# EmaMule/2D-to-3D-Style-Transfer

Measured on AMD Instinct MI355X. Metric: style-transfer iters/sec (512x512, 8 views, cow_mesh), higher is better.
Workload: dtype f32; 1 GPU; BASELINE.json configs[1]: cow_mesh + Style_1, 512x512, 8 views/GPU/iter, texture-only optimisation, white backgrounds (second_approach loop body); texture=512x512, targets_hoisted=content renders + content features + style Grams, parallelism=views sharded dp1, RCCL all-reduce of the texture gradient

## Files before the change

2d-to-3d-style-transfer_amd/csrc/flat.hip:

```cpp
#include "common.h"

namespace {

typedef unsigned u32x4 __attribute__((ext_vector_type(4)));
typedef unsigned u32x2 __attribute__((ext_vector_type(2)));

__global__ __launch_bounds__(256) void flat_v0_kernel(const float *__restrict__ img, const float *__restrict__ color, int S,
                                                      int total4, uint8_t *__restrict__ v0) {
    const int i = blockIdx.x * 256 + threadIdx.x;
    if (i >= total4) return;
    const int per = (S * S) >> 2;
    const int n = i / per, r = i - n * per;
    u32x4 d = u32x4{0u, 0u, 0u, 0u};
#pragma unroll
    for (int c = 0; c < 3; ++c) {
        const u32x4 q = *reinterpret_cast<const u32x4 *>(img + ((size_t)(n * 3 + c) * per + r) * 4);
        d |= q ^ __float_as_uint(color[c]);
    }
    reinterpret_cast<unsigned *>(v0)[i] = (d[0] ? 1u : 0u) | (d[1] ? 0x100u : 0u) | (d[2] ? 0x10000u : 0u) | (d[3] ? 0x1000000u : 0u);
}

__global__ __launch_bounds__(256) void flat_v2_kernel(const uint8_t *__restrict__ v0, int S, int total4, uint8_t *__restrict__ v2) {
    const int i = blockIdx.x * 256 + threadIdx.x;
    if (i >= total4) return;
    const int Sh = S >> 1, q4 = Sh >> 2;
    const int x4 = i % q4, y = (i / q4) % Sh, n = i / (q4 * Sh);
    const int c0 = 8 * x4;
    unsigned w[4] = {0u, 0u, 0u, 0u};
#pragma unroll
    for (int dy = -2; dy <= 5; ++dy) {
        const int yy = 4 * (y >> 1) + dy;
        if (yy < 0 || yy >= S) continue;
        const uint8_t *row = v0 + ((size_t)n * S + yy) * S + c0;
        const u32x2 m = *reinterpret_cast<const u32x2 *>(row);
        w[1] |= m[0]; w[2] |= m[1];
        if (c0 > 0) w[0] |= *reinterpret_cast<const unsigned *>(row - 4);
        if (c0 + 8 < S) w[3] |= *reinterpret_cast<const unsigned *>(row + 8);
    }
    unsigned out = 0;
#pragma unroll
    for (int pr = 0; pr < 2; ++pr) {
        unsigned any = 0;
#pragma unroll
        for (int k = 4 * pr + 2; k <= 4 * pr + 9; ++k) any |= (w[k >> 2] >> (8 * (k & 3))) & 0xffu;
        out |= (any ? 0x0101u : 0u) << (16 * pr);
    }
    reinterpret_cast<unsigned *>(v2)[i] = out;
}

struct FlatGeo {
    int tiles_x, tiles_y, rows, cols;
};

__global__ __launch_bounds__(256) void flat_flags_kernel(const uint8_t *__restrict__ v2, int S, FlatGeo g1, FlatGeo g2, int t1, int t2,
                                                         int total, uint8_t *__restrict__ flags) {
    const int i = blockIdx.x * 4 + (threadIdx.x >> 6), lane = threadIdx.x & 63;
    if (i >= total) return;
    const int Sh = S >> 1;
    const int launch = i < t1 ? 0 : (i < t1 + t2 ? 1 : 2);
    const FlatGeo g = launch == 0 ? FlatGeo{g1.tiles_x, g1.tiles_y, g1.rows >> 1, g1.cols >> 1} : g2;
    const int t = launch == 0 ? i : (launch == 1 ? i - t1 : i - t1 - t2);
    const int per_img = g.tiles_x * g.tiles_y;
    const int n = t / per_img, r = t - n * per_img;
    const int ty = r / g.tiles_x, tx = r - ty * g.tiles_x;
    const int x0 = tx * g.cols, y0 = ty * g.rows;
    const int margin = launch == 0 ? 0 : (launch == 1 ? 1 : 5);
    const int ya = max(0, y0 - margin), yb = min(Sh - 1, y0 + g.rows - 1 + margin);
    const int xa = max(0, x0 - margin), xb = min(Sh - 1, x0 + g.cols - 1 + margin);
    const int w = xb - xa + 1, count = (yb - ya + 1) * w;
    const uint8_t *base = v2 + (size_t)n * Sh * Sh;
    unsigned any = 0;
    for (int k = lane; k < count; k += 64) {
        const int y = ya + k / w, x = xa + k % w;
        any |= base[(size_t)y * Sh + x];
    }
    const bool vary = __any(any != 0);
    if (lane == 0) flags[i] = vary ? 1 : 0;
}

struct FlatLists {
    int *list[3], *map[3];
};

__global__ __launch_bounds__(1024) void flat_lists_kernel(const uint8_t *__restrict__ flags, FlatGeo g1, FlatGeo g2, int t1, int t2,
                                                          FlatLists out, int *__restrict__ counts) {
    __shared__ int scan[1024];
    __shared__ int rep[81];
    const int launch = blockIdx.x, tid = threadIdx.x;
    const uint8_t *__restrict__ f = flags + (launch == 0 ? 0 : (launch == 1 ? t1 : t1 + t2));
    const FlatGeo g = launch == 0 ? g1 : g2;
    const int total = launch == 0 ? t1 : t2;
    int *__restrict__ list = out.list[launch];
    int *__restrict__ map = out.map[launch];
    const int per = (total + 1023) / 1024;
    const int lo = min(total, tid * per), hi = min(total, lo + per);
    struct Walk { int ty, tx; };
    const int r0 = lo % (g.tiles_x * g.tiles_y);
    const Walk w0{r0 / g.tiles_x, r0 % g.tiles_x};
    auto cls = [&](const Walk &w) {
        return ((min(w.ty, 2) * 3 + min(g.tiles_y - 1 - w.ty, 2)) * 3 + min(w.tx, 2)) * 3 + min(g.tiles_x - 1 - w.tx, 2);
    };
    auto step = [&](Walk &w) {
        if (++w.tx == g.tiles_x) { w.tx = 0; if (++w.ty == g.tiles_y) w.ty = 0; }
    };
    unsigned long long fm = 0;
    if (per <= 64)
        for (int t = lo; t < hi; ++t) fm |= (unsigned long long)(f[t] ? 1 : 0) << (t - lo);
    auto varying = [&](int t) { return per <= 64 ? (int)((fm >> (t - lo)) & 1ull) : (int)f[t]; };
    if (tid < 81) rep[tid] = 0x7fffffff;
    __syncthreads();
    Walk w = w0;
    for (int t = lo; t < hi; ++t, step(w)) {
        const int c = cls(w);
        if (!varying(t) && t < *(volatile int *)&rep[c]) atomicMin(&rep[c], t);
    }
    __syncthreads();
    int cnt = 0;
    w = w0;
    for (int t = lo; t < hi; ++t, step(w)) cnt += (varying(t) || rep[cls(w)] == t) ? 1 : 0;
    scan[tid] = cnt;
    __syncthreads();
    for (int d = 1; d < 1024; d <<= 1) {
        const int v = tid >= d ? scan[tid - d] : 0;
        __syncthreads();
        scan[tid] += v;
        __syncthreads();
    }
    int o = scan[tid] - cnt;
    w = w0;
    for (int t = lo; t < hi; ++t, step(w)) {
        const int rp = rep[cls(w)];
        const bool listed = varying(t) || rp == t;
        if (listed) list[o++] = t;
        map[t] = listed ? -1 : rp;
    }
    if (tid == 1023) counts[launch] = scan[1023];
}

struct FillTile { int n, y, x; };
__device__ __forceinline__ void fill_block(char *__restrict__ base, int esize, int C, int c0, int Hh, int Ww, int br, int bc,
                                           FillTile dst, FillTile src, int tid) {
    const int row_chunks = (bc * esize) >> 4;
    const int chunks = 16 * br * row_chunks;
    for (int k = tid; k < chunks; k += 256) {
        const int q = k % row_chunks, r = (k / row_chunks) % br, c = c0 + k / (row_chunks * br);
        const size_t so = ((((size_t)src.n * C + c) * Hh + src.y * br + r) * Ww + src.x * bc) * esize + 16 * q;
        const size_t d_o = ((((size_t)dst.n * C + c) * Hh + dst.y * br + r) * Ww + dst.x * bc) * esize + 16 * q;
        *reinterpret_cast<u32x4 *>(base + d_o) = *reinterpret_cast<const u32x4 *>(base + so);
    }
}

__global__ __launch_bounds__(256) void flat_fill_kernel(const int *__restrict__ map, float *__restrict__ y, float *__restrict__ yp,
                                                        uint8_t *__restrict__ yidx, int C, int H, int W, FlatGeo g, int total) {
    const int t = blockIdx.x;
    const int rp = map[t];
    if (rp < 0 || rp >= total) return;
    const int per_img = g.tiles_x * g.tiles_y;
    const int tr = t % per_img, rr = rp % per_img;
    const FillTile dst{t / per_img, tr / g.tiles_x, tr % g.tiles_x}, src{rp / per_img, rr / g.tiles_x, rr % g.tiles_x};
    const int c0 = blockIdx.y * 16, tid = threadIdx.x;
    if (y) fill_block(reinterpret_cast<char *>(y), 4, C, c0, H, W, g.rows, g.cols, dst, src, tid);
    if (yp) fill_block(reinterpret_cast<char *>(yp), 4, C, c0, H >> 1, W >> 1, g.rows >> 1, g.cols >> 1, dst, src, tid);
    if (yidx) fill_block(reinterpret_cast<char *>(yidx), 1, C, c0, H >> 1, W >> 1, g.rows >> 1, g.cols >> 1, dst, src, tid);
}

int geo_of(int H, int W, FlatGeo *g) {
    int rows = 0, cols = 0;
    if (!st3d_wino43_tile_geometry(H, W, &rows, &cols)) return 0;
    *g = FlatGeo{W / cols, H / rows, rows, cols};
    return 1;
}

}

extern "C" int st3d_flat_levels(int S) { return (S >= 64 && (S % 64) == 0) ? 3 : 0; }

extern "C" int st3d_flat_tiles(int N, int S, int launch) {
    FlatGeo g;
    if (N <= 0 || st3d_flat_levels(S) == 0 || launch < 0 || launch > 2) return 0;
    const int R = launch == 0 ? S : S / 2;
    if (!geo_of(R, R, &g)) return 0;
    return N * g.tiles_x * g.tiles_y;
}

extern "C" size_t st3d_flat_workspace_bytes(int N, int S) {
    if (N <= 0 || st3d_flat_levels(S) == 0) return 0;
    return (size_t)N * S * S + (size_t)N * (S / 2) * (S / 2) + (size_t)st3d_flat_tiles(N, S, 0) + 2 * (size_t)st3d_flat_tiles(N, S, 1);
}

extern "C" int st3d_flat_build(const float *imgs, const float *color, int N, int S, int levels, void *workspace, size_t workspace_bytes,
                               int *list1, int *map1, int *list2, int *map2, int *list3, int *map3, int *counts, st3d_stream_t stream) {
    ST3D_CHECK_ARG(imgs && color && workspace && counts && N > 0);
    ST3D_CHECK_ARG(levels >= 1 && levels <= st3d_flat_levels(S));
    ST3D_CHECK_ARG(((uintptr_t)imgs & 15) == 0 && ((uintptr_t)workspace & 15) == 0);
    ST3D_CHECK_ARG((long)N * S * S < (1L << 31));
    ST3D_CHECK_ARG(workspace_bytes >= st3d_flat_workspace_bytes(N, S));
    ST3D_CHECK_ARG(list1 && map1 && (levels < 2 || (list2 && map2)) && (levels < 3 || (list3 && map3)));
    hipStream_t s = st3d::as_stream(stream);
    FlatGeo g1, g2;
    geo_of(S, S, &g1);
    geo_of(S / 2, S / 2, &g2);
    const int t1 = N * g1.tiles_x * g1.tiles_y, t2 = N * g2.tiles_x * g2.tiles_y;
    uint8_t *v0 = reinterpret_cast<uint8_t *>(workspace);
    uint8_t *v2 = v0 + (size_t)N * S * S;
    uint8_t *flags = v2 + (size_t)N * (S / 2) * (S / 2);
    const int n0 = N * S * S / 4, n2 = N * (S / 2) * (S / 2) / 4;
    flat_v0_kernel<<<st3d::cdiv(n0, 256), 256, 0, s>>>(imgs, color, S, n0, v0);
    ST3D_LAUNCH_CHECK();
    flat_v2_kernel<<<st3d::cdiv(n2, 256), 256, 0, s>>>(v0, S, n2, v2);
    ST3D_LAUNCH_CHECK();
    const int total = t1 + (levels - 1) * t2;
    flat_flags_kernel<<<st3d::cdiv(total, 4), 256, 0, s>>>(v2, S, g1, g2, t1, t2, total, flags);
    ST3D_LAUNCH_CHECK();
    FlatLists out{{list1, list2, list3}, {map1, map2, map3}};
    flat_lists_kernel<<<levels, 1024, 0, s>>>(flags, g1, g2, t1, t2, out, counts);
    ST3D_LAUNCH_CHECK();
    return ST3D_OK;
}

extern "C" int st3d_flat_fill(const int *tile_map, float *y, float *y_pooled, uint8_t *pool_idx, int N, int C, int H, int W,
                              st3d_stream_t stream) {
    ST3D_CHECK_ARG(tile_map && (y || y_pooled) && (!pool_idx || y_pooled));
    ST3D_CHECK_ARG(N > 0 && C > 0 && (C % 16) == 0);
    ST3D_CHECK_ARG((((uintptr_t)y | (uintptr_t)y_pooled | (uintptr_t)pool_idx) & 15) == 0);
    FlatGeo g;
    ST3D_CHECK_ARG(geo_of(H, W, &g));
    const long total = (long)N * g.tiles_x * g.tiles_y;
    ST3D_CHECK_ARG(total < (1L << 31) && C / 16 < 65536);
    flat_fill_kernel<<<dim3((unsigned)total, (unsigned)(C / 16)), 256, 0, st3d::as_stream(stream)>>>(tile_map, y, y_pooled, pool_idx, C, H,
                                                                                                  W, g, (int)total);
    ST3D_LAUNCH_CHECK();
    return ST3D_OK;
}
```

2d-to-3d-style-transfer_amd/csrc/loss.hip:

```cpp
#include "common.h"

namespace {

constexpr int NPART = 1024;

__device__ __forceinline__ float wave_sum(float v) {
#pragma unroll
    for (int o = 32; o > 0; o >>= 1) v += __shfl_down(v, o, 64);
    return v;
}

__device__ __forceinline__ void block_store_partial(float v, float *partials) {
    __shared__ float s[4];
    v = wave_sum(v);
    if ((threadIdx.x & 63) == 0) s[threadIdx.x >> 6] = v;
    __syncthreads();
    if (threadIdx.x == 0) partials[blockIdx.x] = (s[0] + s[1]) + (s[2] + s[3]);
}

__global__ __launch_bounds__(256) void sqdiff_kernel(const float *__restrict__ a, const float *__restrict__ b, size_t n,
                                                     size_t nb, float *__restrict__ D, float *__restrict__ partials) {
    float acc = 0.f;
    const size_t stride = (size_t)gridDim.x * blockDim.x;
    for (size_t i = (size_t)blockIdx.x * blockDim.x + threadIdx.x; i < n; i += stride) {
        const float d = a[i] - b[nb == n ? i : i % nb];
        if (D) D[i] = d;
        acc += d * d;
    }
    block_store_partial(acc, partials);
}

__global__ __launch_bounds__(256) void finish_kernel(const float *__restrict__ partials, int np, float scale,
                                                     float *__restrict__ out) {
    __shared__ double s[256];
    double v = 0.0;
    for (int i = threadIdx.x; i < np; i += 256) v += (double)partials[i];
    s[threadIdx.x] = v;
    __syncthreads();
    for (int o = 128; o > 0; o >>= 1) {
        if ((int)threadIdx.x < o) s[threadIdx.x] += s[threadIdx.x + o];
        __syncthreads();
    }
    if (threadIdx.x == 0) out[0] = out[0] + (float)(s[0] * (double)scale);
}

struct MultiArgs {
    const float *a[8]; const float *b[8]; float *D[8];
    size_t n[8], nb[8];
    float scale[8];
    int slot[8], first_block[9], count;
};

__global__ __launch_bounds__(256) void sqdiff_multi_kernel(const MultiArgs m, float *__restrict__ partials) {
    int k = 0;
    while (k + 1 < m.count && (int)blockIdx.x >= m.first_block[k + 1]) ++k;
    const int lb = blockIdx.x - m.first_block[k], gsz = m.first_block[k + 1] - m.first_block[k];
    const float *a = m.a[k], *b = m.b[k];
    float *D = m.D[k];
    const size_t n = m.n[k], nb = m.nb[k];
    float acc = 0.f;
    const size_t stride = (size_t)gsz * blockDim.x;
    for (size_t i = (size_t)lb * blockDim.x + threadIdx.x; i < n; i += stride) {
        const float d = a[i] - b[nb == n ? i : i % nb];
        if (D) D[i] = d;
        acc += d * d;
    }
    __shared__ float s[4];
    acc = wave_sum(acc);
    if ((threadIdx.x & 63) == 0) s[threadIdx.x >> 6] = acc;
    __syncthreads();
    if (threadIdx.x == 0) partials[(size_t)k * NPART + lb] = (s[0] + s[1]) + (s[2] + s[3]);
}

__global__ __launch_bounds__(256) void finish_multi_kernel(const MultiArgs m, const float *__restrict__ partials, float *__restrict__ out,
                                                           int zero_first, int combine, float sw, float cw) {
    __shared__ double s[256];
    __shared__ float acc3[3];
    if (threadIdx.x < 3) acc3[threadIdx.x] = zero_first ? 0.f : out[threadIdx.x];
    __syncthreads();
    for (int k = 0; k < m.count; ++k) {
        const int np = m.first_block[k + 1] - m.first_block[k];
        double v = 0.0;
        for (int i = threadIdx.x; i < np; i += 256) v += (double)partials[(size_t)k * NPART + i];
        s[threadIdx.x] = v;
        __syncthreads();
        for (int o = 128; o > 0; o >>= 1) {
            if ((int)threadIdx.x < o) s[threadIdx.x] += s[threadIdx.x + o];
            __syncthreads();
        }
        if (threadIdx.x == 0) acc3[m.slot[k]] = acc3[m.slot[k]] + (float)(s[0] * (double)m.scale[k]);
        __syncthreads();
    }
    if (threadIdx.x == 0) {
        if (combine) acc3[0] = cw * acc3[1] + sw * acc3[2];
        out[0] = acc3[0]; out[1] = acc3[1]; out[2] = acc3[2];
    }
}

__global__ __launch_bounds__(256) void axpy_diff_kernel(const float *__restrict__ a, const float *__restrict__ b, size_t n,
                                                        float coef, int accumulate, int gate, float *__restrict__ g) {
    const size_t stride = (size_t)gridDim.x * blockDim.x;
    for (size_t i = (size_t)blockIdx.x * blockDim.x + threadIdx.x; i < n; i += stride) {
        const float ai = a[i];
        const float v = coef * (ai - b[i]);
        const float t = accumulate ? g[i] + v : v;
        g[i] = (gate && ai <= 0.f) ? 0.f : t;
    }
}

__global__ __launch_bounds__(256) void masked_mse_kernel(const float *__restrict__ r, const float *__restrict__ t,
                                                         const float *__restrict__ m, int B, size_t HW, float coef,
                                                         float *__restrict__ gr, float *__restrict__ partials) {
    float acc = 0.f;
    const size_t n = (size_t)B * 3 * HW;
    const size_t stride = (size_t)gridDim.x * blockDim.x;
    for (size_t i = (size_t)blockIdx.x * blockDim.x + threadIdx.x; i < n; i += stride) {
        const size_t b = i / (3 * HW), p = i % HW;
        const float mk = m[b * HW + p];
        const float d = r[i] * mk - t[i] * mk;
        acc += d * d;
        if (gr) gr[i] = coef * d * mk;
    }
    block_store_partial(acc, partials);
}

__global__ __launch_bounds__(256) void adam_kernel(float *__restrict__ p, const float *__restrict__ g,
                                                   float *__restrict__ m, float *__restrict__ v, size_t n,
                                                   float step_size, float bc2_sqrt, float b1, float b2, float eps) {
    const size_t stride = (size_t)gridDim.x * blockDim.x;
    for (size_t i = (size_t)blockIdx.x * blockDim.x + threadIdx.x; i < n; i += stride) {
        const float gi = g[i];
        const float mi = m[i] + (gi - m[i]) * (1.0f - b1);
        const float vi = v[i] * b2 + (1.0f - b2) * gi * gi;
        m[i] = mi;
        v[i] = vi;
        const float denom = sqrtf(vi) / bc2_sqrt + eps;
        p[i] = p[i] - step_size * (mi / denom);
    }
}


__global__ __launch_bounds__(256) void tv_kernel(const float *__restrict__ img, const float *__restrict__ mask, int B, int C,
                                                 int H, int W, float *__restrict__ partials) {
    float acc = 0.f, macc = 0.f;
    const size_t HW = (size_t)H * W, n = (size_t)B * C * HW;
    const size_t stride = (size_t)gridDim.x * blockDim.x;
    for (size_t i = (size_t)blockIdx.x * blockDim.x + threadIdx.x; i < n; i += stride) {
        const size_t bc = i / HW, p = i - bc * HW, b = bc / C;
        const int y = (int)(p / W), x = (int)(p - (size_t)y * W);
        const float *mb = mask + b * HW;
        const float a = img[i], m = mb[p];
        if (y + 1 < H) acc += fabsf(a - img[i + W]) * (m * mb[p + W]);
        if (x + 1 < W) acc += fabsf(a - img[i + 1]) * (m * mb[p + 1]);
        if (bc - b * C == 0) macc += m;
    }
    __shared__ float s2[4];
    macc = wave_sum(macc);
    if ((threadIdx.x & 63) == 0) s2[threadIdx.x >> 6] = macc;
    block_store_partial(acc, partials);
    if (threadIdx.x == 0) partials[NPART + blockIdx.x] = (s2[0] + s2[1]) + (s2[2] + s2[3]);
}

__global__ __launch_bounds__(256) void tv_finish_kernel(const float *__restrict__ partials, int np, float *__restrict__ out) {
    __shared__ double s[256], sm[256];
    double v = 0.0, m = 0.0;
    for (int i = threadIdx.x; i < np; i += 256) { v += (double)partials[i]; m += (double)partials[NPART + i]; }
    s[threadIdx.x] = v; sm[threadIdx.x] = m;
    __syncthreads();
    for (int o = 128; o > 0; o >>= 1) {
        if ((int)threadIdx.x < o) { s[threadIdx.x] += s[threadIdx.x + o]; sm[threadIdx.x] += sm[threadIdx.x + o]; }
        __syncthreads();
    }
    if (threadIdx.x == 0) { out[0] = (float)(s[0] / sm[0]); out[1] = (float)sm[0]; }
}

__device__ __forceinline__ float sgn(float v) { return v > 0.f ? 1.f : (v < 0.f ? -1.f : 0.f); }

__global__ __launch_bounds__(256) void tv_grad_kernel(const float *__restrict__ img, const float *__restrict__ mask, int B, int C,
                                                      int H, int W, const float *__restrict__ loss_and_msum,
                                                      float *__restrict__ g) {
    const size_t HW = (size_t)H * W, n = (size_t)B * C * HW;
    const float inv = 1.0f / loss_and_msum[1];
    const size_t stride = (size_t)gridDim.x * blockDim.x;
    for (size_t i = (size_t)blockIdx.x * blockDim.x + threadIdx.x; i < n; i += stride) {
        const size_t bc = i / HW, p = i - bc * HW, b = bc / C;
        const int y = (int)(p / W), x = (int)(p - (size_t)y * W);
        const float *mb = mask + b * HW;
        const float a = img[i], m = mb[p];
        float d = 0.f;
        if (y + 1 < H) d += sgn(a - img[i + W]) * (m * mb[p + W]);
        if (y > 0) d -= sgn(img[i - W] - a) * (mb[p - W] * m);
        if (x + 1 < W) d += sgn(a - img[i + 1]) * (m * mb[p + 1]);
        if (x > 0) d -= sgn(img[i - 1] - a) * (mb[p - 1] * m);
        g[i] = d * inv;
    }
}

__global__ __launch_bounds__(256) void range_kernel(const float *__restrict__ t, size_t n, float *__restrict__ g,
                                                    float *__restrict__ partials) {
    float acc = 0.f;
    const size_t stride = (size_t)gridDim.x * blockDim.x;
    for (size_t i = (size_t)blockIdx.x * blockDim.x + threadIdx.x; i < n; i += stride) {
        const float v = t[i];
        acc += __builtin_elementwise_maximum(v - 1.0f, 0.f) + __builtin_elementwise_maximum(-v, 0.f);
        if (g) g[i] = v > 1.0f ? 1.0f : (v < 0.f ? -1.0f : 0.f);
    }
    block_store_partial(acc, partials);
}

inline int grid_for(size_t n) {
    size_t b = (n + 255) / 256;
    return (int)(b < 1 ? 1 : (b > NPART ? NPART : b));
}

}

extern "C" int st3d_reduce_partials(void) { return NPART; }

int st3d::finish_partials(const float *partials, int np, float scale, float *loss_out, hipStream_t stream) {
    finish_kernel<<<1, 256, 0, stream>>>(partials, np, scale, loss_out);
    ST3D_LAUNCH_CHECK();
    return ST3D_OK;
}

extern "C" int st3d_sqdiff_sum(const float *a, const float *b, size_t n, size_t nb, float scale, float *D, float *partials,
                               float *loss_out, st3d_stream_t stream) {
    ST3D_CHECK_ARG(a && b && partials && loss_out);
    ST3D_CHECK_ARG(n > 0 && nb > 0 && n % nb == 0);
    hipStream_t s = st3d::as_stream(stream);
    const int gsz = grid_for(n);
    sqdiff_kernel<<<gsz, 256, 0, s>>>(a, b, n, nb, D, partials);
    ST3D_LAUNCH_CHECK();
    finish_kernel<<<1, 256, 0, s>>>(partials, gsz, scale, loss_out);
    ST3D_LAUNCH_CHECK();
    return ST3D_OK;
}

extern "C" int st3d_sqdiff_sum_multi(const st3d_sqdiff_item *items, int count, float *partials, float *loss_out3, int zero_first,
                                     int combine, float style_weight, float content_weight, st3d_stream_t stream) {
    ST3D_CHECK_ARG(items && partials && loss_out3 && count > 0 && count <= 8);
    MultiArgs m;
    memset(&m, 0, sizeof(m));
    m.count = count;
    for (int k = 0; k < count; ++k) {
        ST3D_CHECK_ARG(items[k].a && items[k].b && items[k].n > 0 && items[k].nb > 0 && items[k].n % items[k].nb == 0);
        ST3D_CHECK_ARG(items[k].slot >= 0 && items[k].slot <= 2);
        m.a[k] = items[k].a; m.b[k] = items[k].b; m.D[k] = items[k].D;
        m.n[k] = items[k].n; m.nb[k] = items[k].nb; m.scale[k] = items[k].scale; m.slot[k] = items[k].slot;
        m.first_block[k + 1] = m.first_block[k] + grid_for(items[k].n);
    }
    hipStream_t s = st3d::as_stream(stream);
    sqdiff_multi_kernel<<<m.first_block[count], 256, 0, s>>>(m, partials);
    ST3D_LAUNCH_CHECK();
    finish_multi_kernel<<<1, 256, 0, s>>>(m, partials, loss_out3, zero_first, combine, style_weight, content_weight);
    ST3D_LAUNCH_CHECK();
    return ST3D_OK;
}

extern "C" int st3d_axpy_diff(const float *a, const float *b, size_t n, float coef, int accumulate, float *g,
                              st3d_stream_t stream) {
    ST3D_CHECK_ARG(a && b && g && n > 0);
    axpy_diff_kernel<<<grid_for(n), 256, 0, st3d::as_stream(stream)>>>(a, b, n, coef, accumulate, 0, g);
    ST3D_LAUNCH_CHECK();
    return ST3D_OK;
}

extern "C" int st3d_axpy_diff_gated(const float *a, const float *b, size_t n, float coef, int accumulate, float *g,
                                    st3d_stream_t stream) {
    ST3D_CHECK_ARG(a && b && g && n > 0);
    axpy_diff_kernel<<<grid_for(n), 256, 0, st3d::as_stream(stream)>>>(a, b, n, coef, accumulate, 1, g);
    ST3D_LAUNCH_CHECK();
    return ST3D_OK;
}

extern "C" int st3d_masked_mse(const float *rendered, const float *target, const float *mask, int B, int S,
                               float *grad_rendered, float *partials, float *loss_out, st3d_stream_t stream) {
    ST3D_CHECK_ARG(rendered && target && mask && partials && loss_out);
    ST3D_CHECK_ARG(B > 0 && S > 0);
    hipStream_t s = st3d::as_stream(stream);
    const size_t HW = (size_t)S * S, n = (size_t)B * 3 * HW;
    const int gsz = grid_for(n);
    ST3D_HIP(hipMemsetAsync(loss_out, 0, sizeof(float), s));
    masked_mse_kernel<<<gsz, 256, 0, s>>>(rendered, target, mask, B, HW, 2.0f / (float)n, grad_rendered, partials);
    ST3D_LAUNCH_CHECK();
    finish_kernel<<<1, 256, 0, s>>>(partials, gsz, 1.0f / (float)n, loss_out);
    ST3D_LAUNCH_CHECK();
    return ST3D_OK;
}

extern "C" int st3d_adam_step(float *param, const float *grad, float *exp_avg, float *exp_avg_sq, size_t n, int step,
                              float lr, float beta1, float beta2, float eps, st3d_stream_t stream) {
    ST3D_CHECK_ARG(param && grad && exp_avg && exp_avg_sq);
    ST3D_CHECK_ARG(n > 0 && step >= 1);
    const double bc1 = 1.0 - pow((double)beta1, (double)step);
    const double bc2 = 1.0 - pow((double)beta2, (double)step);
    const float step_size = (float)((double)lr / bc1);
    const float bc2_sqrt = (float)sqrt(bc2);
    adam_kernel<<<grid_for(n), 256, 0, st3d::as_stream(stream)>>>(param, grad, exp_avg, exp_avg_sq, n, step_size, bc2_sqrt,
                                                                 beta1, beta2, eps);
    ST3D_LAUNCH_CHECK();
    return ST3D_OK;
}

extern "C" int st3d_tv_loss(const float *images, const float *masks, int B, int C, int H, int W, float *partials,
                            float *loss_and_mask_sum, float *grad_images, st3d_stream_t stream) {
    ST3D_CHECK_ARG(images && masks && partials && loss_and_mask_sum);
    ST3D_CHECK_ARG(B > 0 && C > 0 && H > 0 && W > 0);
    hipStream_t s = st3d::as_stream(stream);
    const size_t n = (size_t)B * C * H * W;
    const int gsz = grid_for(n);
    tv_kernel<<<gsz, 256, 0, s>>>(images, masks, B, C, H, W, partials);
    ST3D_LAUNCH_CHECK();
    tv_finish_kernel<<<1, 256, 0, s>>>(partials, gsz, loss_and_mask_sum);
    ST3D_LAUNCH_CHECK();
    if (grad_images) {
        tv_grad_kernel<<<gsz, 256, 0, s>>>(images, masks, B, C, H, W, loss_and_mask_sum, grad_images);
        ST3D_LAUNCH_CHECK();
    }
    return ST3D_OK;
}

extern "C" int st3d_range_loss(const float *values, size_t n, float *partials, float *loss_out, float *grad,
                               st3d_stream_t stream) {
    ST3D_CHECK_ARG(values && partials && loss_out && n > 0);
    hipStream_t s = st3d::as_stream(stream);
    const int gsz = grid_for(n);
    ST3D_HIP(hipMemsetAsync(loss_out, 0, sizeof(float), s));
    range_kernel<<<gsz, 256, 0, s>>>(values, n, grad, partials);
    ST3D_LAUNCH_CHECK();
    finish_kernel<<<1, 256, 0, s>>>(partials, gsz, 1.0f, loss_out);
    ST3D_LAUNCH_CHECK();
    return ST3D_OK;
}
```

Measured before the change: 127.5 iter/s (one iter = 8 views of 512x512: render + VGG-19 fwd/bwd + Gram/content loss + Adam).

## Fuse flat-region detection into bitmap front kernel and persistent tile fill

Replaces the v0/v2/flags kernel chain with one tiled front kernel that builds a per-image bitmask of non-background quads directly from the render. Tile flags are then computed inside the list kernel from the bitmap, which is staged in shared memory when it fits, and the block scan now uses wave shuffles. The tile fill kernel becomes a grid-strided persistent kernel that reuses loaded source tiles and uses nontemporal stores. The loss sqdiff loop is unrolled by four to issue more loads in flight. Together these cut launches and intermediate traffic, but add complexity and risk in the bit indexing and fill scheduling.

```diff
diff --git a/2d-to-3d-style-transfer_amd/csrc/flat.hip b/2d-to-3d-style-transfer_amd/csrc/flat.hip
--- a/2d-to-3d-style-transfer_amd/csrc/flat.hip
+++ b/2d-to-3d-style-transfer_amd/csrc/flat.hip
@@ -3,165 +3,232 @@
 namespace {
 
 typedef unsigned u32x4 __attribute__((ext_vector_type(4)));
-typedef unsigned u32x2 __attribute__((ext_vector_type(2)));
-
-__global__ __launch_bounds__(256) void flat_v0_kernel(const float *__restrict__ img, const float *__restrict__ color, int S,
-                                                      int total4, uint8_t *__restrict__ v0) {
-    const int i = blockIdx.x * 256 + threadIdx.x;
-    if (i >= total4) return;
-    const int per = (S * S) >> 2;
-    const int n = i / per, r = i - n * per;
-    u32x4 d = u32x4{0u, 0u, 0u, 0u};
-#pragma unroll
-    for (int c = 0; c < 3; ++c) {
-        const u32x4 q = *reinterpret_cast<const u32x4 *>(img + ((size_t)(n * 3 + c) * per + r) * 4);
-        d |= q ^ __float_as_uint(color[c]);
-    }
-    reinterpret_cast<unsigned *>(v0)[i] = (d[0] ? 1u : 0u) | (d[1] ? 0x100u : 0u) | (d[2] ? 0x10000u : 0u) | (d[3] ? 0x1000000u : 0u);
-}
-
-__global__ __launch_bounds__(256) void flat_v2_kernel(const uint8_t *__restrict__ v0, int S, int total4, uint8_t *__restrict__ v2) {
-    const int i = blockIdx.x * 256 + threadIdx.x;
-    if (i >= total4) return;
-    const int Sh = S >> 1, q4 = Sh >> 2;
-    const int x4 = i % q4, y = (i / q4) % Sh, n = i / (q4 * Sh);
-    const int c0 = 8 * x4;
-    unsigned w[4] = {0u, 0u, 0u, 0u};
-#pragma unroll
-    for (int dy = -2; dy <= 5; ++dy) {
-        const int yy = 4 * (y >> 1) + dy;
-        if (yy < 0 || yy >= S) continue;
-        const uint8_t *row = v0 + ((size_t)n * S + yy) * S + c0;
-        const u32x2 m = *reinterpret_cast<const u32x2 *>(row);
-        w[1] |= m[0]; w[2] |= m[1];
-        if (c0 > 0) w[0] |= *reinterpret_cast<const unsigned *>(row - 4);
-        if (c0 + 8 < S) w[3] |= *reinterpret_cast<const unsigned *>(row + 8);
-    }
-    unsigned out = 0;
-#pragma unroll
-    for (int pr = 0; pr < 2; ++pr) {
-        unsigned any = 0;
-#pragma unroll
-        for (int k = 4 * pr + 2; k <= 4 * pr + 9; ++k) any |= (w[k >> 2] >> (8 * (k & 3))) & 0xffu;
-        out |= (any ? 0x0101u : 0u) << (16 * pr);
-    }
-    reinterpret_cast<unsigned *>(v2)[i] = out;
+typedef unsigned long long u64;
+
+constexpr int kFrontEdge = 64;
+constexpr int kFrontRows = kFrontEdge + 4;
+constexpr int kFrontQuads = kFrontEdge / 4 + 2;
+constexpr int kFrontThreads = 1024;
+constexpr int kMapWords = 4096;
+
+__host__ __device__ inline int row_words(int bw) { return (bw + 63) >> 6; }
+
+__global__ __launch_bounds__(kFrontThreads) void flat_front_kernel(const float *__restrict__ img, const float *__restrict__ color, int S,
+                                                         uint16_t *__restrict__ bits16) {
+    __shared__ uint8_t v0[kFrontRows][kFrontQuads + 2];
+    const int tid = threadIdx.x, tiles = S / kFrontEdge;
+    const int tx = blockIdx.x % tiles, ty = (blockIdx.x / tiles) % tiles, n = blockIdx.x / (tiles * tiles);
+    const int y0 = kFrontEdge * ty - 2, x0 = kFrontEdge * tx - 4;
+    const unsigned c0 = __float_as_uint(color[0]), c1 = __float_as_uint(color[1]), c2 = __float_as_uint(color[2]);
+    const size_t plane = (size_t)S * S;
+    const float *base = img + (size_t)n * 3 * plane;
+    constexpr int kItems = kFrontRows * kFrontQuads, kTrips = (kItems + kFrontThreads - 1) / kFrontThreads;
+    u32x4 px[kTrips][3];
+#pragma unroll
+    for (int j = 0; j < kTrips; ++j) {
+        const int i = tid + kFrontThreads * j;
+        const int row = i / kFrontQuads, q = i - row * kFrontQuads;
+        const float *p = base + (size_t)min(max(y0 + row, 0), S - 1) * S + min(max(x0 + 4 * q, 0), S - 4);
+#pragma unroll
+        for (int c = 0; c < 3; ++c) px[j][c] = *reinterpret_cast<const u32x4 *>(p + c * plane);
+    }
+#pragma unroll
+    for (int j = 0; j < kTrips; ++j) {
+        const int i = tid + kFrontThreads * j;
+        const int row = i / kFrontQuads, q = i - row * kFrontQuads;
+        const int y = y0 + row, x = x0 + 4 * q;
+        const bool inside = y >= 0 && y < S && x >= 0 && x < S;
+        const u32x4 d = (px[j][0] ^ c0) | (px[j][1] ^ c1) | (px[j][2] ^ c2);
+        const unsigned nib = (d[0] ? 1u : 0u) | (d[1] ? 2u : 0u) | (d[2] ? 4u : 0u) | (d[3] ? 8u : 0u);
+        if (i < kItems) v0[row][q] = (uint8_t)(inside ? nib : 0u);
+    }
+    __syncthreads();
+    if (tid >= 256) return;
+    const int yb = tid >> 4, xb = tid & 15;
+    unsigned any = 0;
+#pragma unroll
+    for (int r = 0; r < 8; ++r) {
+        const uint8_t *row = v0[4 * yb + r];
+        any |= (row[xb] & 0xcu) | row[xb + 1] | (row[xb + 2] & 0x3u);
+    }
+    const u64 bits = __ballot(any != 0);
+    const int lane = tid & 63;
+    if ((lane & 15) == 0) {
+        const int bw = S >> 2, pieces = 4 * row_words(bw);
+        uint16_t *row = bits16 + ((size_t)n * bw + 16 * ty + yb) * pieces;
+        row[tx] = (uint16_t)(bits >> lane);
+        if (tx == tiles - 1)
+            for (int j = tiles; j < pieces; ++j) row[j] = 0;
+    }
 }
 
 struct FlatGeo {
     int tiles_x, tiles_y, rows, cols;
 };
 
-__global__ __launch_bounds__(256) void flat_flags_kernel(const uint8_t *__restrict__ v2, int S, FlatGeo g1, FlatGeo g2, int t1, int t2,
-                                                         int total, uint8_t *__restrict__ flags) {
-    const int i = blockIdx.x * 4 + (threadIdx.x >> 6), lane = threadIdx.x & 63;
-    if (i >= total) return;
-    const int Sh = S >> 1;
-    const int launch = i < t1 ? 0 : (i < t1 + t2 ? 1 : 2);
-    const FlatGeo g = launch == 0 ? FlatGeo{g1.tiles_x, g1.tiles_y, g1.rows >> 1, g1.cols >> 1} : g2;
-    const int t = launch == 0 ? i : (launch == 1 ? i - t1 : i - t1 - t2);
-    const int per_img = g.tiles_x * g.tiles_y;
-    const int n = t / per_img, r = t - n * per_img;
-    const int ty = r / g.tiles_x, tx = r - ty * g.tiles_x;
+__device__ __forceinline__ u64 cols_bits(const u64 *row, int xa, int xb) {
+    const int j = xa >> 6, sh = xa & 63, n = xb - xa + 1;
+    u64 v = row[j] >> sh;
+    if (sh + n > 64) v |= row[j + 1] << (64 - sh);
+    return v & (n >= 64 ? ~0ull : (1ull << n) - 1ull);
+}
+
+__device__ __forceinline__ bool tile_varies(const u64 *maps, int S, int launch, FlatGeo g, int n, int ty, int tx) {
+    const int Sh = S >> 1, bw = S >> 2, W = row_words(bw);
     const int x0 = tx * g.cols, y0 = ty * g.rows;
     const int margin = launch == 0 ? 0 : (launch == 1 ? 1 : 5);
-    const int ya = max(0, y0 - margin), yb = min(Sh - 1, y0 + g.rows - 1 + margin);
-    const int xa = max(0, x0 - margin), xb = min(Sh - 1, x0 + g.cols - 1 + margin);
-    const int w = xb - xa + 1, count = (yb - ya + 1) * w;
-    const uint8_t *base = v2 + (size_t)n * Sh * Sh;
-    unsigned any = 0;
-    for (int k = lane; k < count; k += 64) {
-        const int y = ya + k / w, x = xa + k % w;
-        any |= base[(size_t)y * Sh + x];
-    }
-    const bool vary = __any(any != 0);
-    if (lane == 0) flags[i] = vary ? 1 : 0;
+    const int ya = max(0, y0 - margin) >> 1, yb = min(Sh - 1, y0 + g.rows - 1 + margin) >> 1;
+    const int xa = max(0, x0 - margin) >> 1, xb = min(Sh - 1, x0 + g.cols - 1 + margin) >> 1;
+    const u64 *rows = maps + (size_t)n * bw * W;
+    u64 any = 0;
+    for (int y = ya; y <= yb; ++y) any |= cols_bits(rows + y * W, xa, xb);
+    return any != 0;
 }
 
 struct FlatLists {
     int *list[3], *map[3];
 };
 
-__global__ __launch_bounds__(1024) void flat_lists_kernel(const uint8_t *__restrict__ flags, FlatGeo g1, FlatGeo g2, int t1, int t2,
-                                                          FlatLists out, int *__restrict__ counts) {
-    __shared__ int scan[1024];
+template <bool STAGED>
+__global__ __launch_bounds__(1024) void flat_lists_kernel(const u64 *__restrict__ bits, int words, int S, FlatGeo g1, FlatGeo g2, int t1,
+                                                          int t2, FlatLists out, int *__restrict__ counts) {
+    __shared__ int wave_sum[16];
     __shared__ int rep[81];
+    __shared__ u64 staged[STAGED ? kMapWords : 1];
     const int launch = blockIdx.x, tid = threadIdx.x;
-    const uint8_t *__restrict__ f = flags + (launch == 0 ? 0 : (launch == 1 ? t1 : t1 + t2));
+    if (STAGED)
+        for (int i = tid; i < words; i += 1024) staged[i] = bits[i];
+    const u64 *maps = STAGED ? staged : bits;
     const FlatGeo g = launch == 0 ? g1 : g2;
+    const FlatGeo gv = launch == 0 ? FlatGeo{g1.tiles_x, g1.tiles_y, g1.rows >> 1, g1.cols >> 1} : g2;
     const int total = launch == 0 ? t1 : t2;
     int *__restrict__ list = out.list[launch];
     int *__restrict__ map = out.map[launch];
     const int per = (total + 1023) / 1024;
     const int lo = min(total, tid * per), hi = min(total, lo + per);
-    struct Walk { int ty, tx; };
-    const int r0 = lo % (g.tiles_x * g.tiles_y);
-    const Walk w0{r0 / g.tiles_x, r0 % g.tiles_x};
+    struct Walk { int n, ty, tx; };
+    const int per_img = g.tiles_x * g.tiles_y;
+    const int r0 = lo % per_img;
+    const Walk w0{lo / per_img, r0 / g.tiles_x, r0 % g.tiles_x};
     auto cls = [&](const Walk &w) {
         return ((min(w.ty, 2) * 3 + min(g.tiles_y - 1 - w.ty, 2)) * 3 + min(w.tx, 2)) * 3 + min(g.tiles_x - 1 - w.tx, 2);
     };
     auto step = [&](Walk &w) {
-        if (++w.tx == g.tiles_x) { w.tx = 0; if (++w.ty == g.tiles_y) w.ty = 0; }
+        if (++w.tx == g.tiles_x) { w.tx = 0; if (++w.ty == g.tiles_y) { w.ty = 0; ++w.n; } }
     };
-    unsigned long long fm = 0;
-    if (per <= 64)
-        for (int t = lo; t < hi; ++t) fm |= (unsigned long long)(f[t] ? 1 : 0) << (t - lo);
-    auto varying = [&](int t) { return per <= 64 ? (int)((fm >> (t - lo)) & 1ull) : (int)f[t]; };
+    auto flag = [&](const Walk &w) { return tile_varies(maps, S, launch, gv, w.n, w.ty, w.tx) ? 1 : 0; };
     if (tid < 81) rep[tid] = 0x7fffffff;
     __syncthreads();
+    unsigned long long fm = 0;
     Walk w = w0;
+    if (per <= 64)
+        for (int t = lo; t < hi; ++t, step(w)) fm |= (unsigned long long)flag(w) << (t - lo);
+    auto varying = [&](int t, const Walk &w) { return per <= 64 ? (int)((fm >> (t - lo)) & 1ull) : flag(w); };
+    w = w0;
     for (int t = lo; t < hi; ++t, step(w)) {
         const int c = cls(w);
-        if (!varying(t) && t < *(volatile int *)&rep[c]) atomicMin(&rep[c], t);
+        if (!varying(t, w) && t < *(volatile int *)&rep[c]) atomicMin(&rep[c], t);
     }
     __syncthreads();
     int cnt = 0;
     w = w0;
-    for (int t = lo; t < hi; ++t, step(w)) cnt += (varying(t) || rep[cls(w)] == t) ? 1 : 0;
-    scan[tid] = cnt;
+    for (int t = lo; t < hi; ++t, step(w)) cnt += (varying(t, w) || rep[cls(w)] == t) ? 1 : 0;
+    const int lane = tid & 63, wave = tid >> 6;
+    int incl = cnt;
+#pragma unroll
+    for (int d = 1; d < 64; d <<= 1) {
+        const int v = __shfl_up(incl, d);
+        if (lane >= d) incl += v;
+    }
+    if (lane == 63) wave_sum[wave] = incl;
     __syncthreads();
-    for (int d = 1; d < 1024; d <<= 1) {
-        const int v = tid >= d ? scan[tid - d] : 0;
-        __syncthreads();
-        scan[tid] += v;
-        __syncthreads();
-    }
-    int o = scan[tid] - cnt;
+    int before = 0, all = 0;
+#pragma unroll
+    for (int k = 0; k < 16; ++k) {
+        const int v = wave_sum[k];
+        before += k < wave ? v : 0;
+        all += v;
+    }
+    int o = before + incl - cnt;
     w = w0;
     for (int t = lo; t < hi; ++t, step(w)) {
         const int rp = rep[cls(w)];
-        const bool listed = varying(t) || rp == t;
+        const bool listed = varying(t, w) || rp == t;
         if (listed) list[o++] = t;
         map[t] = listed ? -1 : rp;
     }
-    if (tid == 1023) counts[launch] = scan[1023];
-}
-
-struct FillTile { int n, y, x; };
-__device__ __forceinline__ void fill_block(char *__restrict__ base, int esize, int C, int c0, int Hh, int Ww, int br, int bc,
-                                           FillTile dst, FillTile src, int tid) {
+    if (tid == 0) counts[launch] = all;
+}
+
+__device__ __forceinline__ unsigned chunk_offset(int k, int esize, int Hh, int Ww, int br, int bc) {
     const int row_chunks = (bc * esize) >> 4;
-    const int chunks = 16 * br * row_chunks;
-    for (int k = tid; k < chunks; k += 256) {
-        const int q = k % row_chunks, r = (k / row_chunks) % br, c = c0 + k / (row_chunks * br);
-        const size_t so = ((((size_t)src.n * C + c) * Hh + src.y * br + r) * Ww + src.x * bc) * esize + 16 * q;
-        const size_t d_o = ((((size_t)dst.n * C + c) * Hh + dst.y * br + r) * Ww + dst.x * bc) * esize + 16 * q;
-        *reinterpret_cast<u32x4 *>(base + d_o) = *reinterpret_cast<const u32x4 *>(base + so);
-    }
+    const int q = k % row_chunks, r = (k / row_chunks) % br, c = k / (row_chunks * br);
+    return (unsigned)(((c * Hh + r) * Ww) * esize + 16 * q);
+}
+
+struct FillOrigin { unsigned y16, p16; };
+__device__ __forceinline__ FillOrigin fill_origin(int t, int cg, int C, int H, int W, FlatGeo g) {
+    const int per_img = g.tiles_x * g.tiles_y;
+    const int n = t / per_img, r = t - n * per_img, ty = r / g.tiles_x, tx = r - ty * g.tiles_x;
+    const size_t plane = (size_t)n * C + 16 * cg;
+    return FillOrigin{(unsigned)(((plane * H + ty * g.rows) * W + tx * g.cols) >> 2),
+                      (unsigned)(((plane * (H >> 1) + ty * (g.rows >> 1)) * (W >> 1) + tx * (g.cols >> 1)) >> 2)};
 }
 
 __global__ __launch_bounds__(256) void flat_fill_kernel(const int *__restrict__ map, float *__restrict__ y, float *__restrict__ yp,
-                                                        uint8_t *__restrict__ yidx, int C, int H, int W, FlatGeo g, int total) {
-    const int t = blockIdx.x;
-    const int rp = map[t];
-    if (rp < 0 || rp >= total) return;
-    const int per_img = g.tiles_x * g.tiles_y;
-    const int tr = t % per_img, rr = rp % per_img;
-    const FillTile dst{t / per_img, tr / g.tiles_x, tr % g.tiles_x}, src{rp / per_img, rr / g.tiles_x, rr % g.tiles_x};
-    const int c0 = blockIdx.y * 16, tid = threadIdx.x;
-    if (y) fill_block(reinterpret_cast<char *>(y), 4, C, c0, H, W, g.rows, g.cols, dst, src, tid);
-    if (yp) fill_block(reinterpret_cast<char *>(yp), 4, C, c0, H >> 1, W >> 1, g.rows >> 1, g.cols >> 1, dst, src, tid);
-    if (yidx) fill_block(reinterpret_cast<char *>(yidx), 1, C, c0, H >> 1, W >> 1, g.rows >> 1, g.cols >> 1, dst, src, tid);
+                                                        uint8_t *__restrict__ yidx, int C, int H, int W, FlatGeo g, int total, int groups) {
+    const int tid = threadIdx.x, lane = tid & 63, Hh = H >> 1, Wh = W >> 1, br = g.rows >> 1, bc = g.cols >> 1;
+    unsigned oy[4];
+#pragma unroll
+    for (int j = 0; j < 4; ++j) oy[j] = chunk_offset(tid + 256 * j, 4, H, W, g.rows, g.cols);
+    const unsigned op = chunk_offset(tid, 4, Hh, Wh, br, bc), oi = chunk_offset(lane, 1, Hh, Wh, br, bc);
+    const bool has_idx = yidx && tid < 64;
+    char *const by = reinterpret_cast<char *>(y), *const bp = reinterpret_cast<char *>(yp), *const bi = reinterpret_cast<char *>(yidx);
+    const u32x4 zero = u32x4{0u, 0u, 0u, 0u};
+    u32x4 vy[4] = {zero, zero, zero, zero}, vp = zero, vi = zero;
+    int held_rp = -1, held_cg = -1;
+    const int units = total * groups, stride = gridDim.x;
+    for (int u0 = blockIdx.x; u0 < units; u0 += 64 * stride) {
+        const int ul = u0 + lane * stride;
+        int rpl = -1, cgl = 0;
+        FillOrigin dl{0u, 0u};
+        if (ul < units) {
+            const int t = ul / groups;
+            cgl = ul - t * groups;
+            rpl = map[t];
+            dl = fill_origin(t, cgl, C, H, W, g);
+        }
+        u64 todo = __ballot(rpl >= 0 && rpl < total);
+        while (todo) {
+            const int i = __ffsll((long long)todo) - 1;
+            todo &= todo - 1;
+            const int rp = __builtin_amdgcn_readlane(rpl, i), cg = __builtin_amdgcn_readlane(cgl, i);
+            const size_t dy = (size_t)(unsigned)__builtin_amdgcn_readlane((int)dl.y16, i) << 4;
+            const size_t dp = (size_t)(unsigned)__builtin_amdgcn_readlane((int)dl.p16, i) << 4;
+            if (rp != held_rp || cg != held_cg) {
+                const FillOrigin src = fill_origin(rp, cg, C, H, W, g);
+                const size_t sy = (size_t)src.y16 << 4, sp = (size_t)src.p16 << 4;
+                if (y) {
+#pragma unroll
+                    for (int j = 0; j < 4; ++j) vy[j] = *reinterpret_cast<const u32x4 *>(by + sy + oy[j]);
+                }
+                if (yp) vp = *reinterpret_cast<const u32x4 *>(bp + sp + op);
+                if (has_idx) vi = *reinterpret_cast<const u32x4 *>(bi + (sp >> 2) + oi);
+#pragma unroll
+                for (int j = 0; j < 4; ++j) asm volatile("" : "+v"(vy[j]));
+                asm volatile("" : "+v"(vp));
+                asm volatile("" : "+v"(vi));
+                held_rp = rp;
+                held_cg = cg;
+            }
+            if (y) {
+#pragma unroll
+                for (int j = 0; j < 4; ++j) __builtin_nontemporal_store(vy[j], reinterpret_cast<u32x4 *>(by + dy + oy[j]));
+            }
+            if (yp) __builtin_nontemporal_store(vp, reinterpret_cast<u32x4 *>(bp + dp + op));
+            if (has_idx) __builtin_nontemporal_store(vi, reinterpret_cast<u32x4 *>(bi + (dp >> 2) + oi));
+        }
+    }
 }
 
 int geo_of(int H, int W, FlatGeo *g) {
@@ -185,7 +252,7 @@
 
 extern "C" size_t st3d_flat_workspace_bytes(int N, int S) {
     if (N <= 0 || st3d_flat_levels(S) == 0) return 0;
-    return (size_t)N * S * S + (size_t)N * (S / 2) * (S / 2) + (size_t)st3d_flat_tiles(N, S, 0) + 2 * (size_t)st3d_flat_tiles(N, S, 1);
+    return (size_t)N * (S / 4) * row_words(S / 4) * sizeof(u64);
 }
 
 extern "C" int st3d_flat_build(const float *imgs, const float *color, int N, int S, int levels, void *workspace, size_t workspace_bytes,
@@ -201,19 +268,15 @@
     geo_of(S, S, &g1);
     geo_of(S / 2, S / 2, &g2);
     const int t1 = N * g1.tiles_x * g1.tiles_y, t2 = N * g2.tiles_x * g2.tiles_y;
-    uint8_t *v0 = reinterpret_cast<uint8_t *>(workspace);
-    uint8_t *v2 = v0 + (size_t)N * S * S;
-    uint8_t *flags = v2 + (size_t)N * (S / 2) * (S / 2);
-    const int n0 = N * S * S / 4, n2 = N * (S / 2) * (S / 2) / 4;
-    flat_v0_kernel<<<st3d::cdiv(n0, 256), 256, 0, s>>>(imgs, color, S, n0, v0);
-    ST3D_LAUNCH_CHECK();
-    flat_v2_kernel<<<st3d::cdiv(n2, 256), 256, 0, s>>>(v0, S, n2, v2);
-    ST3D_LAUNCH_CHECK();
-    const int total = t1 + (levels - 1) * t2;
-    flat_flags_kernel<<<st3d::cdiv(total, 4), 256, 0, s>>>(v2, S, g1, g2, t1, t2, total, flags);
+    u64 *bits = reinterpret_cast<u64 *>(workspace);
+    const int tiles = S / kFrontEdge, words = N * (S / 4) * row_words(S / 4);
+    flat_front_kernel<<<N * tiles * tiles, kFrontThreads, 0, s>>>(imgs, color, S, reinterpret_cast<uint16_t *>(bits));
     ST3D_LAUNCH_CHECK();
     FlatLists out{{list1, list2, list3}, {map1, map2, map3}};
-    flat_lists_kernel<<<levels, 1024, 0, s>>>(flags, g1, g2, t1, t2, out, counts);
+    if (words <= kMapWords)
+        flat_lists_kernel<true><<<levels, 1024, 0, s>>>(bits, words, S, g1, g2, t1, t2, out, counts);
+    else
+        flat_lists_kernel<false><<<levels, 1024, 0, s>>>(bits, words, S, g1, g2, t1, t2, out, counts);
     ST3D_LAUNCH_CHECK();
     return ST3D_OK;
 }
@@ -226,9 +289,16 @@
     FlatGeo g;
     ST3D_CHECK_ARG(geo_of(H, W, &g));
     const long total = (long)N * g.tiles_x * g.tiles_y;
-    ST3D_CHECK_ARG(total < (1L << 31) && C / 16 < 65536);
-    flat_fill_kernel<<<dim3((unsigned)total, (unsigned)(C / 16)), 256, 0, st3d::as_stream(stream)>>>(tile_map, y, y_pooled, pool_idx, C, H,
-                                                                                                  W, g, (int)total);
+    const int groups = C / 16;
+    const long units = total * groups;
+    ST3D_CHECK_ARG((long)H * W * 64 < (1L << 31) && (long)N * C * H * W / 4 < (1L << 32) && units < (1L << 30));
+    int dev = 0, cus = 0;
+    if (hipGetDevice(&dev) != hipSuccess || hipDeviceGetAttribute(&cus, hipDeviceAttributeMultiprocessorCount, dev) != hipSuccess || cus <= 0) cus = 256;
+    long wgs = (8L * cus + groups - 1) / groups * groups;
+    if (const char *e = getenv("ST3D_FLAT_FILL_WGS")) { if (atol(e) > 0) wgs = atol(e); }
+    if (wgs > units) wgs = units;
+    if (wgs > (1L << 24)) wgs = 1L << 24;
+    flat_fill_kernel<<<(unsigned)wgs, 256, 0, st3d::as_stream(stream)>>>(tile_map, y, y_pooled, pool_idx, C, H, W, g, (int)total, groups);
     ST3D_LAUNCH_CHECK();
     return ST3D_OK;
 }
diff --git a/2d-to-3d-style-transfer_amd/csrc/loss.hip b/2d-to-3d-style-transfer_amd/csrc/loss.hip
--- a/2d-to-3d-style-transfer_amd/csrc/loss.hip
+++ b/2d-to-3d-style-transfer_amd/csrc/loss.hip
@@ -60,7 +60,23 @@
     const size_t n = m.n[k], nb = m.nb[k];
     float acc = 0.f;
     const size_t stride = (size_t)gsz * blockDim.x;
-    for (size_t i = (size_t)lb * blockDim.x + threadIdx.x; i < n; i += stride) {
+    size_t i = (size_t)lb * blockDim.x + threadIdx.x;
+    for (; i + 3 * stride < n; i += 4 * stride) {
+        float av[4], bv[4];
+#pragma unroll
+        for (int j = 0; j < 4; ++j) {
+            const size_t e = i + j * stride;
+            av[j] = a[e];
+            bv[j] = b[nb == n ? e : e % nb];
+        }
+#pragma unroll
+        for (int j = 0; j < 4; ++j) {
+            const float d = av[j] - bv[j];
+            if (D) D[i + j * stride] = d;
+            acc += d * d;
+        }
+    }
+    for (; i < n; i += stride) {
         const float d = a[i] - b[nb == n ? i : i % nb];
         if (D) D[i] = d;
         acc += d * d;
```

Result: no change. 127.9 iter/s (one iter = 8 views of 512x512: render + VGG-19 fwd/bwd + Gram/content loss + Adam), median of 6 (+0.4%).
